# wreuven/h264-scroll-encoder

Hardware: AMD Instinct MI355X
Metric: composed frames/sec (1280x720, 360x360 dyn) at 1/2/4/8 GPU; bit-exact vs CPU (higher is better)
Workload: dtype u8; 1 GPU; BASELINE config 3: 256 concurrent 1280x720 streams + 360x360 synthetic dynamic rect (4x4 int transform + quant + CAVLC), composer_write_scroll_frame semantics; resolution=1280x720, streams_per_gpu=256, parallelism=static stream shard x1, no RCCL

## Files before the change

### h264-scroll-encoder_amd/csrc/dyn_kernels.hip

```cpp
#include <hip/hip_runtime.h>

#include <stdint.h>
#include <mutex>

#include "dyn_device.h"
#include "dyn_engine.h"
#include "nal_ctx.h"
#include "stage_util.h"

using namespace scroll;
using namespace scroll::dyn;
using namespace scroll::stage;

namespace {

__constant__ Tabs g_tabs = SCROLL_DYN_TABS;
constexpr Tabs k_tabs = SCROLL_DYN_TABS;
__constant__ PTabs g_ptabs = make_ptabs(k_tabs);
__device__ uint32_t g_tzrb[TZRB_N];
struct QpPair {
    QParams l, c;
};
struct QpTab {
    QpPair q[QP_MAX + 1];
};
constexpr QpTab make_qptab()
{
    QpTab T{};
    for (int i = 0; i <= QP_MAX; ++i) T.q[i] = QpPair{qparams(i), qparams(qp_chroma(i))};
// ... 4 lines not shown
__global__ __launch_bounds__(256) void k_tzrb_init()
{
    const int i = blockIdx.x * 256 + threadIdx.x;
    if (i < TZRB_N) g_tzrb[i] = i < 65536 ? tzrb_entry(g_tabs, (uint32_t)i, 16) : tzrb_entry(g_tabs, (uint32_t)(i - 65536), 15);
}

__device__ inline void load_ptabs(PTabs &dst, int t, int nthr)
{
    constexpr int N = (int)(sizeof(PTabs) / 16);
    static_assert(sizeof(PTabs) % 16 == 0, "PTabs copies as uint4");
    for (int i = t; i < N; i += nthr) reinterpret_cast<uint4 *>(&dst)[i] = reinterpret_cast<const uint4 *>(&g_ptabs)[i];
}

constexpr int HEAD_MAX = 160;
constexpr int HDR_MAX = 1024;
constexpr int OBUF = 6400;

constexpr uint32_t DF_OVER = 1u, DF_GENERAL = 2u, DF_HANDOFF = 4u;
constexpr uint64_t HANDOFF_TICKS = 5000000ull;
constexpr uint64_t HANDOFF_GAP = 100000ull;
constexpr uint32_t DF_EPSLOW = 0x100u;
constexpr uint32_t DF_FIXED = 0x200u;

constexpr int EPC_ROW = 256, EPC_STATIC = 4096;

__device__ inline uint32_t ep_data(uint32_t w, uint32_t gi, uint32_t bits)
{
    const uint32_t b0 = 32u * gi;
    if (__builtin_expect(b0 + 32u <= bits, 1)) return w;
    return w | (bits > b0 ? 0xffffffffu >> (bits - b0) : 0xffffffffu);
}

__device__ inline uint32_t ep_run_starts(uint32_t pw, uint32_t w, uint32_t nx, uint32_t gi, uint32_t bits)
{
    uint64_t X = (uint64_t)ep_data(w, gi, bits) << 32 | ep_data(nx, gi + 1u, bits);
    X |= X << 1;
    X |= X << 2;
    X |= X << 4;
    X |= X << 8;
    X |= X << 6;
    const uint32_t z22 = ~(uint32_t)(X >> 32);
    return z22 & ((ep_data(w, gi, bits) >> 1) | (pw << 31));
}

__device__ inline bool ep_quick(uint32_t w, uint32_t nx)
{
    uint32_t y = w | w << 1;
    y |= y << 2;
    y |= y << 4;
    y |= y << 8;
    y |= y << 6;
    const uint32_t tz = w ? (uint32_t)__builtin_ctz(w) : 32u, lz = nx ? (uint32_t)__builtin_clz(nx) : 32u;
    return (~y & 0xffe00000u) != 0u || tz + lz >= 22u;
}

__device__ inline void flush_window(const uint32_t *buf, uint32_t n, uint32_t p0, bool last, uint32_t *out,
                                    uint32_t *ncand, uint32_t *cg, uint32_t cmax, int t, int nthr)
{
    const int lane = t & 63;
    for (uint32_t i0 = 0; i0 < n; i0 += (uint32_t)nthr) {
        const uint32_t i = i0 + (uint32_t)t;
        bool q = false;
        if (i < n) {
            const uint32_t w = buf[i];
            out[p0 + i] = w;
            q = ep_quick(w, i + 1 < n ? buf[i + 1] : (last ? 0xffffffffu : 0u));
        }
        const uint64_t m = __builtin_amdgcn_ballot_w64(q);
        if (m) {
            uint32_t base = 0;
            if (lane == (int)__builtin_ctzll(m)) base = atomicAdd(ncand, (uint32_t)__builtin_popcountll(m));
            base = (uint32_t)__shfl((int)base, (int)__builtin_ctzll(m), 64);
            const uint32_t k = base + (uint32_t)__builtin_popcountll(m & ((1ull << lane) - 1ull));
            if (q && k < cmax) cg[1 + k] = p0 + i;
        }
    }
}

__device__ inline uint32_t ld32(const uint8_t *p) { return *reinterpret_cast<const uint32_t *>(p); }

constexpr int NPC = DYN_PIECES;

__device__ inline void put_body(uint2 *BL, uint2 *BH, size_t i, uint4 v, bool hi)
{
    BL[i] = make_uint2(v.x, v.y);
    if (hi) BH[i] = make_uint2(v.z, v.w);
}

__device__ inline uint4 get_body(const uint2 *BL, const uint2 *BH, size_t i, bool hi)
{
    const uint2 a = BL[i], b = hi ? BH[i] : make_uint2(0u, 0u);
    return make_uint4(a.x, a.y, b.x, b.y);
}

__device__ inline int rec_of(int q, int pc, int ndt)
{
    return pc < 16 ? 16 * q + pc : (pc < 18 ? 24 * ndt + 2 * q + (pc - 16) : 16 * ndt + 8 * q + (pc - 18));
// ... 562 lines not shown
        uint32_t e = 0u;
        if (gen) {
            const uint32_t k = atomicAdd(&ctr[1], 1u);
            if (k < g.gen_cap) {
                DF->rbsp_bytes = k;
                ctr[DYN_CTR_LIST + k] = (uint32_t)((size_t)s * ld_fr + f);
                e = DF_GENERAL;
            } else {
                e = DF_OVER;
            }
        }
        DF->err = e;
        DF->ep = (uint32_t)qpy;
    }
}

constexpr int GW = 64;
#ifndef SCROLL_GBUF_WORDS
#define SCROLL_GBUF_WORDS 256
#endif
constexpr int GBUF_WORDS = SCROLL_GBUF_WORDS;

struct StaticFixed {
    uint32_t ncand;
    uint32_t buf[GBUF_WORDS];
    uint64_t hhi[12], hlo[12];
    uint4 pat[12];
    uint32_t hlen[12];
    int32_t head_over;
    int32_t wo[8], wl[8], wv[8];
    uint32_t moff[DYN_STATIC_ROWS + 1];
};

__global__ __launch_bounds__(GW) void k_dyn_static(const DevStream *__restrict__ st,
                                                   const NalDesc *__restrict__ nal, int ld_nal,
                                                   const PlanPending *__restrict__ pend,
                                                   const DynFrame *__restrict__ dfr, int ld_fr, DynGeom g,
                                                   uint32_t *__restrict__ rowstage, uint32_t *__restrict__ gbits)
{
    __shared__ StaticFixed L;
    constexpr int SR = DYN_STATIC_ROWS;
    const Rect R{g.x0, g.y0, g.w, g.h};
    const int nA = max(1, (R.y0 + SR - 1) / SR);
    const int gi = (int)blockIdx.x >= nA ? (int)blockIdx.x + R.h : (int)blockIdx.x;
    const int ng = g.ngroups, f = blockIdx.y, s = blockIdx.z, t = threadIdx.x;
    const size_t nb = (size_t)s * ld_fr + f;
    const DynFrame df = dfr[nb];
    const int j = df.nal;
    if (j < 0) return;
    const bool first = gi == 0, last = gi == ng - 1;
    if (t < 8) {
        L.wo[t] = pend[s].wo[t];
        L.wl[t] = pend[s].wl[t];
        L.wv[t] = pend[s].wv[t];
    }
    if (t == 0) {
        L.head_over = 0;
        L.ncand = 0;
    }
    const DevStream *S = st + s;
    const NalDesc d = nal[(size_t)s * ld_nal + j];
    wave_sync();
    NalCtx c = nal_ctx(S, d, L.wo, L.wl, L.wv);
    c.qpd = (int)df.ep - QP_DEFAULT;
    const HeadCtx H = head_ctx(c);
    const int mbw = H.mbw, mbh = c.h / 16;
    int ra, rb;
    if (gi < nA) {
        ra = gi * SR;
        rb = min(ra + SR, R.y0);
    } else {
        ra = R.y0 + R.h + (gi - nA - R.h) * SR;
        rb = min(ra + SR, mbh);
    }
    uint32_t F = 0;
    if (first) {
        CountSink hc{0};
        emit_slice_header(hc, c);
        F = hc.n;
    }
    if (t < 12) {
// ... 97 lines not shown
                    const uint32_t w0 = wi == 0 ? P.x : (wi == 1 ? P.y : (wi == 2 ? P.z : P.w));
                    const uint32_t w1 = wi == 0 ? P.y : (wi == 1 ? P.z : (wi == 2 ? P.w : 0u));
                    uint32_t v = sh ? __builtin_amdgcn_alignbit(w0, w1, 32u - sh) : w0;
                    v &= k >= 32u ? 0xffffffffu : ~(0xffffffffu >> k);
                    acc |= v >> (b - W0);
                    b += k;
                }
                L.buf[i] = acc;
            }
            wave_sync();
            if (first && t == 0 && p0 * 32u < F) {
                WSink hs{win, 0, 0, 0};
                hs.start(0);
                emit_slice_header(hs, c);
                hs.finish();
            }
            if (last && t == 0) {
                WSink sk{win, 0, 0, 0};
                sk.start(bits - 1u);
                sk.put(1, 1);
                sk.finish();
            }
            wave_sync();
            flush_window(L.buf, n, p0, p0 + n >= nw, out, &L.ncand,
                         rowstage + nb * g.rs_frame_words + rs_runs_words(g, nA, gi), EPC_STATIC - 1, t, GW);
            wave_sync();
            continue;
        }
        const int ea = max(cnt_le(32u * p0) - 1, 0), eb = min(cnt_le(32u * (p0 + n) - 1u), ne);
        const int nm = eb * mbw;
        for (int m = ea * mbw + t; m < nm; m += GW) {
            const int rr = (int)div_m((uint32_t)m, m_mbw), col = m - rr * mbw, rw = ra + rr;
            uint32_t off = L.moff[rr];
            WSink sk{win, 0, 0, 0};
            if (!head_over) {
                const int b3 = H.sel(rw, 0);
                off += col == 0 ? 0u : L.hlen[b3] + 1u + (uint32_t)(col - 1) * (L.hlen[b3 + 1] + 1u);
                if (off >= 32u * (p0 + n)) continue;
                const int cls = b3 + (col == 0 ? 0 : (col == mbw - 1 ? 2 : 1));
                if (off + L.hlen[cls] + 1u <= 32u * p0) continue;
                sk.start(off);
                sk.put_cap(CapSink{L.hhi[cls], L.hlo[cls], L.hlen[cls]});
            } else {
                for (int c2 = 0; c2 < col; ++c2) off += head_bits(rw, c2) + 1u;
                sk.start(off);
                H.put_slow(sk, rw, col);
            }
            sk.put(1, 1);
            sk.finish();
        }
        if (last && t == 0) {
            WSink sk{win, 0, 0, 0};
            sk.start(bits - 1u);
            sk.put(1, 1);
            sk.finish();
        }
        wave_sync();
        flush_window(L.buf, n, p0, p0 + n >= nw, out, &L.ncand,
                     rowstage + nb * g.rs_frame_words + rs_runs_words(g, nA, gi), EPC_STATIC - 1, t, GW);
        wave_sync();
    }
    if (t == 0) rowstage[nb * g.rs_frame_words + rs_runs_words(g, nA, gi)] = L.ncand;
}


__device__ inline CapSink cap_of_msb(uint64_t a, uint64_t b, uint32_t n)
{
    if (n == 0u) return CapSink{0, 0, 0};
    const uint32_t sh = 128u - n;
    if (sh >= 64u) return CapSink{0, a >> (sh - 64u), n};
    if (sh == 0u) return CapSink{a, b, n};
    return CapSink{a >> sh, (b >> sh) | (a << (64u - sh)), n};
}

__device__ inline void put_piece(uint32_t *buf, uint32_t p0, uint32_t n, uint32_t pos, uint32_t tv, uint32_t tl,
                                 uint4 b, uint32_t bl)
{
    const uint32_t tw = tv & low_mask((int)tl);
    const uint32_t c0 = __builtin_amdgcn_alignbit(tw, b.x, tl), c1 = __builtin_amdgcn_alignbit(b.x, b.y, tl);
    const uint32_t c2 = __builtin_amdgcn_alignbit(b.y, b.z, tl), c3 = __builtin_amdgcn_alignbit(b.z, b.w, tl);
    const uint32_t c4 = __builtin_amdgcn_alignbit(b.w, 0u, tl);
    const uint32_t sh = pos & 31u;
    const uint32_t o[6] = {c0 >> sh, __builtin_amdgcn_alignbit(c0, c1, sh), __builtin_amdgcn_alignbit(c1, c2, sh),
                           __builtin_amdgcn_alignbit(c2, c3, sh), __builtin_amdgcn_alignbit(c3, c4, sh),
                           __builtin_amdgcn_alignbit(c4, 0u, sh)};
// ... 43 lines not shown
#define SCROLL_ROW_GB 896
#endif
constexpr int ROW_GB = SCROLL_ROW_GB;

constexpr int ROW_PCD_N = (NPC + 3) & ~3;

struct RowFixed {
    RowTabs ptabs;
    uint32_t pcd[ROW_PCD_N];
    union {
        uint32_t buf[ROW_GB + 4];
        struct {
            uint32_t kc[2][SORT_KEYS];
            uint32_t ovf;
            uint32_t kc_pad[31 - 2 * SORT_KEYS];
            uint32_t lvt[LVT_N];
        };
    };
    uint64_t hhi[12], hlo[12];
    uint32_t hlen[12];
    int32_t wo[8], wl[8], wv[8];
    int32_t head_over;
    uint32_t rt[32];
    uint32_t ncand;
    uint32_t spill;
};

static_assert(2 * SORT_KEYS < 31 && 32 + LVT_N <= ROW_GB, "the sort counts, ovf and the level table share the bit window");
static_assert(ROW_PAD == 4, "RowFixed::buf holds ROW_PAD spare words");
static_assert(sizeof(RowFixed) <= 4992, "eight config-3 row workgroups per CU");

__host__ __device__ inline size_t row_lds_base(int w)
{
    return (size_t)16 * NPC * w + (size_t)4 * (w + 1) + (size_t)2 * (3 * NPC * w) + (size_t)10 * w + 16;
}
#ifndef SCROLL_ROW_GB_WIDE
#define SCROLL_ROW_GB_WIDE 1248
#endif
constexpr int ROW_GB_WIDE = SCROLL_ROW_GB_WIDE;
__host__ __device__ inline size_t row_wide_off(int w) { return (row_lds_base(w) + 15) & ~(size_t)15; }
__host__ __device__ inline bool row_wide_win(int w)
{
    return w > SCROLL_ROW_WIDE && row_wide_off(w) + 4 * (size_t)(ROW_GB_WIDE + ROW_PAD) + sizeof(RowFixed) <= 163840;
}
__host__ __device__ inline size_t row_lds_bytes(int w)
{
    return row_wide_win(w) ? row_wide_off(w) + 4 * (size_t)(ROW_GB_WIDE + ROW_PAD) : row_lds_base(w);
// ... 33 lines not shown
    RowConst C{};
    const PTabs P = make_ptabs(T);
    for (int i = 0; i < 4 * 68; ++i) C.ptabs.ct[i / 68][i % 68] = P.ct[i / 68][i % 68];
    for (int i = 0; i < 12; ++i) C.ptabs.tzdc[i / 4][i % 4] = P.tzdc[i / 4][i % 4];
    for (int i = 0; i < 7 * 16; ++i) C.ptabs.rb[i / 16][i % 16] = P.rb[i / 16][i % 16];
    for (int i = 0; i < NPC; ++i) C.pcd[i] = pc_desc(i);
    const LvTab V = make_lvt();
    for (int i = 0; i < LVT_N; ++i) C.lvt[i] = V.e[i];
    return C;
}
__constant__ RowConst g_rowconst = make_rowconst(k_tabs);
constexpr int ROWC_NV = (int)(sizeof(RowConst) / 16), ROWC_HEAD = (int)(offsetof(RowConst, lvt) / 16);
constexpr int ROWC_GAP = (int)((offsetof(RowFixed, lvt) - offsetof(RowConst, lvt)) / 16);
static_assert(offsetof(RowFixed, ptabs) == 0 && offsetof(RowFixed, pcd) == offsetof(RowConst, pcd) &&
                  offsetof(RowFixed, kc) == offsetof(RowConst, lvt) && offsetof(RowFixed, lvt) % 16 == 0 &&
                  sizeof(RowConst) % 16 == 0 && sizeof(RowConst) == 16 * ROWC_HEAD + 4 * LVT_N,
              "RowConst is RowFixed's head without the sort's words");
static_assert(offsetof(RowFixed, wl) == offsetof(RowFixed, wo) + 32 && offsetof(RowFixed, wv) == offsetof(RowFixed, wo) + 64 &&
                  offsetof(PlanPending, wl) == offsetof(PlanPending, wo) + 32 &&
                  offsetof(PlanPending, wv) == offsetof(PlanPending, wo) + 64,
              "the waypoint table copies as 24 words");

struct EpfLds {
    uint32_t *goff, *gb, *gw, *cw, *cbase, *lst, *cnt;
    uint32_t *ws;
};
__host__ __device__ inline int row_chroma0(int w) { return (16 * w + 63) & ~63; }
__host__ __device__ inline int row_vtasks(int w) { return row_chroma0(w) + 8 * w; }

__host__ __device__ inline int row_threads(int w)
{
    const int nt = row_vtasks(w), np = w > SCROLL_ROW_WIDE ? SCROLL_ROW_NP_WIDE : SCROLL_ROW_NP;
    const int a = (((nt + np - 1) / np) + 63) & ~63;
    const int b = (((nt + ROW_NPMAX - 1) / ROW_NPMAX) + 63) & ~63;
    const int t = a > b ? a : b;
    return t < ROW_MAXT ? t : ROW_MAXT;
}

struct BlkPix {
    uint32_t a[4], b[4], c;
};

__device__ inline __amdgpu_buffer_rsrc_t buf_rsrc(const void *p, uint32_t n)
{
    return __builtin_amdgcn_make_buffer_rsrc(const_cast<void *>(p), (short)0, (int)n, 0x00020000);
}

// ... 171 lines not shown
        const uint32_t rtv = rtg[e < 16 ? 16 * r + e : 16 * g.h + (e < 24 ? 8 * r + e - 16 : 8 * g.h + 8 * r + e - 24)];
        if (k0 == 0) {
            fetch_luma(fo, t, r, g, rtg + 16 * r);
            fo.pb = 0;
            fetch_pass9(fo, 0u, (uint32_t)(16 * w), fs, rb, nx);
            nx.c = 0u;
            L.rt[e] = rtv;
        } else if (k0 == 1) {
            fetch_chroma(fo, t - L0, r, g, csz, rtg + 16 * g.h + 8 * r, rtg + 24 * g.h + 8 * r);
            fo.pb = 0;
            fo_chroma = true;
            fetch_pass9(fo, 0u, (uint32_t)(8 * w), fs, rb, nx);
        }
    }
    if (df.nal < 0 || ((df.err & DF_GENERAL) != 0) != GEN) return;

    uint4 *lv = rdyn;
    uint32_t *moff = reinterpret_cast<uint32_t *>(lv + npc);
    uint16_t *mt = reinterpret_cast<uint16_t *>(moff + w + 1), *lo = mt + npc, *off16 = lo + npc;
    uint16_t *order = off16;
    uint8_t *ta = reinterpret_cast<uint8_t *>(off16 + npc), *cbpa = ta + 8 * w, *codea = cbpa + w;
    uint32_t *mbits = reinterpret_cast<uint32_t *>(ta);

    if (t == 0) L.ncand = 0;
    if (t == 0) L.ovf = 0u;
    if (t < SORT_KEYS) L.kc[0][t] = 0u;
    if (general && wv0 == T - 64) row_copy_tabs(L, s, nb, lane);
    const int qpy = __builtin_amdgcn_readfirstlane((int)df.ep);
    const QParams ql = g_qptab.q[qpy].l, qc = g_qptab.q[qpy].c;
    const HeadSel HS = head_sel(S, a.nal[(size_t)s * a.ld_nal + df.nal]);
    if (!general)
        asm volatile(""
                     :
                     : "s"(HS.a_end), "s"(HS.mbw), "s"(ql.mf0), "s"(ql.mf1), "s"(ql.mf2), "s"(ql.qbits), "s"(ql.qf),
                       "s"(qc.mf0), "s"(qc.mf1), "s"(qc.mf2), "s"(qc.qbits), "s"(qc.qf));

    __syncthreads();
    if (!general) {
        static_assert(ROW_MAXT % 64 == 0, "row_threads gives whole waves: the per-pass step T is a multiple of 64");
        const uint32_t frc = __builtin_amdgcn_readfirstlane((L.rt[16] >> 28) & 7u);
        const int qL = nl > wv0 ? (nl - wv0 + T - 1) / T : 0;
        const int qC = ntv > wv0 ? (ntv - wv0 + T - 1) / T : 0;
        auto issue_l = [&](int q, BlkPix &px) {
            fetch_pass9(fo, (uint32_t)((q - fo.pb) * T), (uint32_t)(16 * w), fs, rb, px);
        };
        auto issue_c = [&](int q, BlkPix &px) {
            if (!fo_chroma) {
// ... 472 lines not shown
            const uint32_t o = off16[i];
            if (o == 0xffffu) continue;
            const int k = div_npc(i), pc = i - k * NPC;
            const uint32_t e = lo[i], mv = mt[i];
            const uint32_t pos = moff[k] + o;
            if (!one && (pos >= 32u * (p0 + n) || pos + (e & LO_LEN) <= 32u * p0)) continue;
            const int nC = (int)(e >> 11) - 1;
            const uint4 bd = lv[i];
            if (!(mv & M_OVF)) {
                if (nC == -1) {
                    if (one) put_piece1(wb, pos, 0u, 0u, bd, e & LO_LEN);
                    else put_piece(wb, p0, n, pos, 0u, 0u, bd, e & LO_LEN);
                } else {
                    uint32_t tv = 0, tl = 0;
                    piece_token(ctab, mv, nC, tv, tl);
                    if (one) put_piece1(wb, pos, tv, tl, bd, mv & 255u);
                    else put_piece(wb, p0, n, pos, tv, tl, bd, mv & 255u);
                }
            } else {
                ovf_put((LdsWords)wb, p0, n, pos, PT, TB, bd, ovf_wide(k, pc), pc, nC);
            }
        }
        __syncthreads();
        flush_window(wb, n, p0, p0 + n >= nw, out, &L.ncand, out + epc, EPC_ROW - 1, t, T);
        __syncthreads();
    }
    if (t == 0 && !lost) out[epc] = L.ncand;
    if (stp && t == 0) {
        stp[5] = __builtin_amdgcn_s_memrealtime();
        stp[6] = bits;
        stp[7] = (uint64_t)(uint32_t)__builtin_amdgcn_s_getreg((31 << 11) | 4);
    }
}

#ifndef SCROLL_EPS_KW
#define SCROLL_EPS_KW 4
#endif
constexpr int EPS_KW = SCROLL_EPS_KW;
static_assert(EPS_KW % 4 == 0, "the EP scan reads 16-byte LDS vectors");
__host__ __device__ inline size_t gtab_bytes(int ng, bool epfix)
{
    return (size_t)4 * (epfix ? 5 * (size_t)ng + 2 : 3 * (size_t)ng + 1);
}
struct GTab {
    uint32_t *goff, *gb, *gw, *cw, *cbase;
};
__device__ inline GTab gtab_of(uint32_t *p, int ng)
{
    GTab T;
    T.goff = p;
    T.gb = p + ng + 1;
    T.gw = T.gb + ng;
    T.cw = T.gw + ng;
    T.cbase = T.cw + ng;
    return T;
}

__device__ inline uint32_t rs_word_span(uint32_t P, int &gg, int ng, uint32_t T, const uint32_t *goff,
                                       const uint32_t *gb, const uint32_t *gw, const uint32_t *fr)
{
    uint32_t acc = 0, filled = 0;
    while (filled < 32u && gg < ng && P + filled < T) {
        const uint32_t lp = P + filled - goff[gg];
        if (lp >= gb[gg]) {
            ++gg;
            continue;
        }
        const uint32_t take = min(32u - filled, gb[gg] - lp);
        const uint32_t *src = fr + gw[gg];
        const uint32_t i = lp >> 5, sh = lp & 31u;
        uint32_t x = src[i];
        if (sh) {
            x <<= sh;
            if (32u - sh < take) x |= src[i + 1] >> (32u - sh);
        }
        x &= take >= 32u ? 0xffffffffu : ~(0xffffffffu >> take);
        acc |= x >> filled;
// ... 22 lines not shown
__device__ inline void scan_load(ScanLoads &L, uint32_t c0, int t, int ng, uint32_t T, const uint32_t *goff,
                                   const uint32_t *gb, const uint32_t *gw, const uint32_t *fr, int &gcarry)
{
    const uint32_t P0 = c0 * 8u + 32u * (uint32_t)t;
    int gg = gcarry;
    while (gg + 1 < ng && goff[gg + 1] <= P0) ++gg;
#pragma unroll
    for (int k = 0; k < EPS_KW; ++k) {
        const uint32_t P = P0 + 32u * NT * (uint32_t)k;
        while (gg + 1 < ng && goff[gg + 1] <= P) ++gg;
        L.g[k] = gg;
        const uint32_t lp = P - goff[gg], i = lp >> 5;
        const uint32_t *src = fr + gw[gg];
        L.x0[k] = P < T && lp < gb[gg] ? src[i] : 0u;
        L.x1[k] = P < T && (lp & 31u) && 32u * (i + 1) < gb[gg] ? src[i + 1] : 0u;
        const bool seam = P < T && gb[gg] - lp < 32u && gg + 1 < ng;
        L.y[k] = seam ? fr[gw[gg + 1]] : 0u;
    }
    gcarry = gg;
}

__device__ inline void rs_table(const uint32_t *gbits, size_t nb, const DynGeom &g, const uint32_t *fr,
                                uint32_t *goff, uint32_t *gb, uint32_t *gw, uint32_t *cw, int t,
                                uint32_t *bad = nullptr, uint32_t *cnt = nullptr)
{
    const int ng = g.ngroups;
    constexpr int SR = DYN_STATIC_ROWS;
    const int nA = max(1, (g.y0 + SR - 1) / SR);
    if (t >= 64) return;
    uint32_t carry = 0;
    for (int g0 = 0; g0 < ng; g0 += 64) {
        const int gi = g0 + t;
        const bool in = gi < ng;
        const bool row = gi >= nA && gi < nA + g.h;
        uint32_t w = (uint32_t)rs_group_words(g, nA, gi), c = (uint32_t)rs_runs_words(g, nA, gi);
        const uint32_t b = in ? gbits[nb * (size_t)ng + gi] : 0u;
        uint32_t m = in && (row || cnt) ? fr[c] : 0u;
        const uint32_t incl = wave_incl_sum(b, t);
        if (in) {
            gb[gi] = b;
            goff[gi] = carry + incl - b;
            if (row && (m & 0x80000000u)) {
                const uint64_t base = ((uint64_t)g.rs_frames - nb) * g.rs_frame_words;
                const uint64_t rel = (uint64_t)(m & 0x7fffffffu) - base;
                if ((m & 0x7fffffffu) >= base && rel % g.rs_spill_words == 0 &&
                    rel / g.rs_spill_words < g.rs_spill_cap) {
                    w = m & 0x7fffffffu;
                    c = w + g.rs_spill_words - EPC_ROW;
                    if (cnt) m = fr[c];
                } else {
                    if (bad) *bad = 1u;
                    m = 0u;
                }
            }
            gw[gi] = w;
            if (cw) cw[gi] = c;
            if (cnt) cnt[gi] = m;
        }
        carry += __shfl(incl, 63, 64);
    }
    if (t == 0) goff[ng] = carry;
}

__device__ inline uint32_t rs_word(uint32_t P, int ng, uint32_t T, const uint32_t *goff, const uint32_t *gb,
                                   const uint32_t *gw, const uint32_t *fr)
{
    if (P >= T) return 0u;
    int gg = rs_group_at(P, ng, goff);
    return rs_word_span(P, gg, ng, T, goff, gb, gw, fr);
}

__device__ inline uint32_t pick9(const uint32_t w[9], uint32_t i)
{
    const uint32_t a = (i & 1u) ? w[1] : w[0], b = (i & 1u) ? w[3] : w[2];
    const uint32_t c = (i & 1u) ? w[5] : w[4], e = (i & 1u) ? w[7] : w[6];
    const uint32_t ab = (i & 2u) ? b : a, ce = (i & 2u) ? e : c;
    const uint32_t r = (i & 4u) ? ce : ab;
    return (i & 8u) ? w[8] : r;
}

// ... 147 lines not shown
    }
    __syncthreads();
    return ep_n;
}

#ifndef SCROLL_EPF_T
#define SCROLL_EPF_T 128
#endif
#ifndef SCROLL_EPF_LIST
#define SCROLL_EPF_LIST 2048
#endif
constexpr int EPF_T = SCROLL_EPF_T;

__device__ inline void ep_put(uint32_t j, bool bm, uint32_t *lst, uint32_t *nlst, uint32_t lcap)
{
    if (bm) {
        atomicOr(&lst[j >> 5], 1u << (j & 31u));
    } else {
        const uint32_t q = atomicAdd(nlst, 1u);
        if (q < lcap) lst[q] = j;
    }
}

__device__ inline void ep_eval_bytes(uint32_t B, uint32_t Bend, uint32_t nin, int ng, uint32_t T,
                                     const uint32_t *goff, const uint32_t *gb, const uint32_t *gw,
                                     const uint32_t *fr, bool bm, uint32_t *lst, uint32_t *nlst, uint32_t lcap)
{
    uint32_t cw = 0, ci = 0xffffffffu;
    auto byte_at = [&](uint32_t i) -> uint32_t {
        if ((i >> 2) != ci) {
            ci = i >> 2;
            cw = rs_word(32u * ci, ng, T, goff, gb, gw, fr);
        }
        return (cw >> (8u * (3u - (i & 3u)))) & 255u;
    };
    int k = 0;
    for (int64_t i = (int64_t)B - 1; i >= 0; --i) {
        if (byte_at((uint32_t)i)) break;
        ++k;
    }
    for (uint32_t i = B; i < nin; ++i) {
        const uint32_t b = byte_at(i);
        if (ep_insert(b, k)) ep_put(i, bm, lst, nlst, lcap);
        if (b == 0) {
            ++k;
        } else {
            if (i >= Bend) break;
            k = 0;
        }
    }
}

__device__ inline int cand_group(uint32_t i, int ng, const uint32_t *cbase)
{
    int lo = 0, hi = ng;
    while (hi - lo > 1) {
        const int mid = (lo + hi) >> 1;
        if (cbase[mid] <= i) lo = mid;
        else hi = mid;
    }
    return lo;
}

template <int NT, int LCAP>
__device__ __attribute__((always_inline)) inline uint32_t ep_list_windows(uint32_t *lst, uint32_t n, uint32_t nin,
                                                                          uint32_t *eplist, uint32_t *ws, int t,
                                                                          int lane, int wave, uint32_t ecap)
{
    const uint32_t ws0 = (n + 4u * NT - 1u) / (4u * NT) * (4u * NT);
    const uint32_t HW = (uint32_t)LCAP - ws0, CH = HW / (uint32_t)NT;
    uint32_t *win = lst + ws0;
    const uint4 *wv = reinterpret_cast<const uint4 *>(win) + (uint32_t)t * (CH / 4u);
    uint32_t base = 0;
    for (uint32_t w0 = 0; w0 < nin; w0 += 32u * HW) {
        for (uint32_t i = (uint32_t)t; i < HW / 4u; i += (uint32_t)NT)
            reinterpret_cast<uint4 *>(win)[i] = make_uint4(0u, 0u, 0u, 0u);
// ... 20 lines not shown
        ex += incl - mine;
        for (uint32_t k = 0; mine && k < CH / 4u; ++k) {
            const uint4 q = wv[k];
            const uint32_t wv4[4] = {q.x, q.y, q.z, q.w};
#pragma unroll
            for (int e = 0; e < 4; ++e)
                for (uint32_t m = wv4[e]; m; m &= m - 1u) {
                    if (ex < ecap)
                        eplist[ex] = w0 + 32u * ((uint32_t)t * CH + 4u * k + (uint32_t)e) + (uint32_t)__builtin_ctz(m);
                    ++ex;
                }
        }
        base += tot;
        __syncthreads();
    }
    return base;
}

template <int NT, int LCAP>
__device__ inline void ep_fix(DevStream *st, DynFrame *DF, size_t nb, int s, const DynGeom &g,
                              const uint32_t *rowstage, const uint32_t *gbits, uint8_t *eps, const EpfLds &E,
                              int t, uint64_t *stp)
{
    static_assert(NT >= 128 && NT % 64 == 0, "ep_fix: one seam wave and at least one candidate wave");
    static_assert(LCAP % (4 * NT) == 0 && LCAP >= 8 * NT, "ep_fix: the bitmap in whole 16-byte chunks per thread");
    auto stamp = [&](int k) {
        if (stp && t == 0) stp[k] = __builtin_amdgcn_s_memrealtime();
    };
    stamp(0);
    uint32_t *goff = E.goff, *gb = E.gb, *gw = E.gw, *cw = E.cw, *cbase = E.cbase, *lst = E.lst;
    uint32_t &nlst = E.cnt[0], &nu = E.cnt[1], &slow = E.cnt[2], &bad = E.cnt[3];
    const uint32_t lcap = LCAP;
    const uint32_t err0 = DF->err;
    if (err0 & (DF_OVER | DF_HANDOFF)) {
        if (t == 0) {
            DF->rbsp_bytes = 0;
            DF->ep = 0;
            DF->err = err0 | DF_FIXED;
            atomicOr((unsigned int *)&st[s].err,
                     (err0 & DF_HANDOFF) ? SCROLL_DEVERR_HANDOFF : SCROLL_DEVERR_DYN);
        }
        return;
    }
    const int ng = g.ngroups;
    constexpr int SR = DYN_STATIC_ROWS;
    const int nA = max(1, (g.y0 + SR - 1) / SR);
    const uint32_t *fr = rowstage + nb * g.rs_frame_words;
    for (uint32_t i = (uint32_t)t; i < lcap / 4u; i += (uint32_t)NT)
        reinterpret_cast<uint4 *>(lst)[i] = make_uint4(0u, 0u, 0u, 0u);
    if (t < 64) {
        if (t == 0) bad = 0u;
        wave_sync();
        rs_table(gbits, nb, g, fr, goff, gb, gw, cw, t, &bad, cbase);
        wave_sync();
        uint32_t carry = 0;
        bool ov = false;
        for (int g0 = 0; g0 < ng; g0 += 64) {
            const int gi = g0 + t;
            const uint32_t c = gi < ng ? cbase[gi] : 0u;
            const uint32_t cmax = (gi >= nA && gi < nA + g.h) ? EPC_ROW - 1u : EPC_STATIC - 1u;
            const uint32_t cc = min(c, cmax);
            const uint32_t incl = wave_incl_sum(cc, t);
            if (gi < ng) cbase[gi] = carry + incl - cc;
            ov |= __builtin_amdgcn_ballot_w64(c > cmax) != 0;
            carry += __shfl(incl, 63, 64);
        }
        if (t == 0) {
            cbase[ng] = carry;
            slow = ov ? 1u : 0u;
            nlst = 0;
        }
    }
    __syncthreads();
    stamp(1);
    if (bad) {
        if (t == 0) {
            DF->err = DF_OVER | DF_FIXED;
            DF->rbsp_bytes = 0;
            DF->ep = 0;
            atomicOr((unsigned int *)&st[s].err, SCROLL_DEVERR_DYN);
        }
        return;
    }
    const uint32_t T = goff[ng];
    const uint32_t nin = (T + 7) >> 3;
    if (((nin + 31u) & ~31u) > g.slot_bytes - DYN_OVF_BYTES) {
        if (t == 0) {
            DF->err = DF_OVER | DF_FIXED;
            DF->rbsp_bytes = 0;
            DF->ep = 0;
            atomicOr((unsigned int *)&st[s].err, SCROLL_DEVERR_DYN);
        }
        return;
    }
    const uint32_t nbw = (nin + 31u) >> 5;
    const bool bm = nbw <= lcap;
    const int wave = t >> 6, lane = t & 63;
    constexpr int NC = NT;
    const uint32_t nc = cbase[ng];
    if (!slow) {
        if (wave == NT / 64 - 1) {
            for (int k = lane; k < ng; k += 64) {
                const uint32_t S = goff[k];
                if (S < T) ep_eval_bytes(S >> 3, (S + 7) >> 3, nin, ng, T, goff, gb, gw, fr, bm, lst, &nlst, lcap);
            }
            if (stp && lane == 0) stp[7] = __builtin_amdgcn_s_memrealtime();
        }
        constexpr int CB = NC >= 192 ? 2 : 4;
        for (uint32_t i0 = 0; i0 < nc; i0 += (uint32_t)(CB * NC)) {
            uint32_t wi[CB], gg[CB];
#pragma unroll
            for (int q = 0; q < CB; ++q) {
                const uint32_t ci = i0 + (uint32_t)(q * NC + t);
                gg[q] = ci < nc ? (uint32_t)cand_group(ci, ng, cbase) : 0u;
                wi[q] = ci < nc ? fr[cw[gg[q]] + 1u + (ci - cbase[gg[q]])] : 0xffffffffu;
            }
            uint32_t pw[CB], w[CB], nx[CB], nwd[CB];
#pragma unroll
            for (int q = 0; q < CB; ++q) {
                const uint32_t *src = fr + gw[gg[q]];
                nwd[q] = (gb[gg[q]] + 31u) >> 5;
                const bool ok = wi[q] < nwd[q];
                pw[q] = ok && wi[q] ? src[wi[q] - 1u] : 0u;
                w[q] = ok ? src[wi[q]] : 0u;
                nx[q] = ok && wi[q] + 1u < nwd[q] ? src[wi[q] + 1u] : 0u;
            }
#pragma unroll
            for (int q = 0; q < CB; ++q) {
                if (wi[q] >= nwd[q]) continue;
                const uint32_t bits = gb[gg[q]], O = goff[gg[q]], x = wi[q];
                const uint32_t *src = fr + gw[gg[q]];
                const uint32_t wd = ep_data(w[q], x, bits);
                const uint32_t nd = x + 1u < nwd[q] ? ep_data(nx[q], x + 1u, bits) : 0xffffffffu;
                uint32_t m = ep_run_starts(pw[q], wd, nd, x, bits);
                while (m) {
                    const uint32_t a = (uint32_t)__builtin_clz(m);
                    m &= ~(0x80000000u >> a);
                    const uint64_t Y = ((uint64_t)wd << 32 | nd) << a;
                    uint32_t e = bits;
                    if (Y) {
                        e = 32u * x + a + (uint32_t)__builtin_clzll(Y);
                    } else {
                        for (uint32_t r = x + 2u; r < nwd[q]; ++r) {
                            const uint32_t v = ep_data(src[r], r, bits);
                            if (v) {
                                e = 32u * r + (uint32_t)__builtin_clz(v);
                                break;
                            }
                        }
                    }
                    const uint32_t A = (O + 32u * x + a + 7u) & ~7u, E2 = O + e;
                    for (uint32_t j = A + 16u; j + 6u <= E2; j += 16u) ep_put(j >> 3, bm, lst, &nlst, lcap);
                }
            }
        }
        stamp(4);
    }
    __syncthreads();
    stamp(2);
    const uint32_t n = nlst;
    uint32_t *eplist = reinterpret_cast<uint32_t *>(eps + nb * eps_stride(g));
    if (slow || (!bm && n > lcap)) {
        static_assert(NT * EPS_KW <= LCAP, "ep_scan's chunk buffer is the position set's LDS");
        __syncthreads();
        const uint32_t ne = ep_scan<NT>(fr, ng, T, goff, gb, gw, lst, reinterpret_cast<int *>(E.ws), nlst, eplist, t, g.ep_cap);
        if (t == 0) {
            DF->err = DF_EPSLOW | DF_FIXED;
            DF->rbsp_bytes = nin;
            DF->ep = ne;
        }
        return;
    }
    constexpr int CW = LCAP / NT;
    if (!bm && n <= lcap - 4u * NT) {
        const uint32_t base = ep_list_windows<NT, LCAP>(lst, n, nin, eplist, E.ws, t, lane, wave, g.ep_cap);
        stamp(3);
// ... 81 lines not shown
#endif
#if SCROLL_EPF_WAVES
#define EPF_ATTR __attribute__((amdgpu_waves_per_eu(SCROLL_EPF_WAVES)))
#else
#define EPF_ATTR
#endif
template <int NT, int LCAP>
__global__ __launch_bounds__(NT) EPF_ATTR void k_dyn_epfix(DevStream *__restrict__ st, DynFrame *__restrict__ dfr,
                                                     int ld_fr, int nframes, DynGeom g,
                                                     const uint32_t *__restrict__ rowstage,
                                                     const uint32_t *__restrict__ gbits, uint8_t *__restrict__ eps,
                                                     uint64_t *__restrict__ stamps)
{
    __shared__ __attribute__((aligned(16))) uint32_t lst[LCAP];
    extern __shared__ uint32_t gdyn[];
    const GTab GT = gtab_of(gdyn, g.ngroups);
    uint32_t *goff = GT.goff, *gb = GT.gb, *gw = GT.gw, *cw = GT.cw, *cbase = GT.cbase;
    __shared__ uint32_t cnt[4], ws[NT / 64];
    const int f = blockIdx.x, s = blockIdx.y, t = threadIdx.x;
    if (f >= nframes) return;
    const size_t nb = (size_t)s * ld_fr + f;
    DynFrame *DF = dfr + nb;
    if (DF->nal < 0) return;
    const EpfLds E{goff, gb, gw, cw, cbase, lst, cnt, ws};
    ep_fix<NT, LCAP>(st, DF, nb, s, g, rowstage, gbits, eps, E, t, stamps ? stamps + ((size_t)s * nframes + f) * 8 : nullptr);
}
constexpr int EPF_BIG_LIST = 8192;
constexpr int EPF_BIG_MBS = 1024;
inline bool epf_big_rect(int64_t mbs)
{
    static const int env = [] {
        const char *e = getenv("SCROLL_EPF_BIG");
        return e ? atoi(e) : -1;
    }();
    return env >= 0 ? env != 0 : mbs > EPF_BIG_MBS;
}

__device__ inline void store16(uint8_t *A, uint64_t p, const uint8_t *src, uint64_t lo, uint64_t hi)
{
    if (p >= lo && p + 16 <= hi) {
        *reinterpret_cast<uint4 *>(A + p) = *reinterpret_cast<const uint4 *>(src);
        return;
    }
    for (int i = 0; i < 16; ++i)
        if (p + i >= lo && p + i < hi) A[p + i] = src[i];
}

// ... 796 lines not shown
```

Before: 3.253 million frames/s.

## Record run edges and candidate words in emulation-prevention records to skip byte-scan seams

Emulation-prevention candidate records now store each candidate's word and next word, plus per-group leading and trailing zero-run lengths, written where the rows and static groups are encoded. The fix kernel then handles group seams as precomputed zero runs spread across all threads, instead of one wave walking bytes serially through rs_word. Most candidates also no longer re-read their neighbouring bitstream words. In exchange, candidate records are three times larger, the LDS table grows, and the seam logic is more intricate and must stay bit-exact.

```diff
diff --git a/h264-scroll-encoder_amd/csrc/dyn_kernels.hip b/h264-scroll-encoder_amd/csrc/dyn_kernels.hip
--- a/h264-scroll-encoder_amd/csrc/dyn_kernels.hip
+++ b/h264-scroll-encoder_amd/csrc/dyn_kernels.hip
@@ -5,6 +5,7 @@
 
 #include "dyn_device.h"
 #include "dyn_engine.h"
+#include "ep_runs.h"
 #include "nal_ctx.h"
 #include "stage_util.h"
 
@@ -55,57 +56,39 @@
 constexpr uint32_t DF_EPSLOW = 0x100u;
 constexpr uint32_t DF_FIXED = 0x200u;
 
-constexpr int EPC_ROW = 256, EPC_STATIC = 4096;
-
-__device__ inline uint32_t ep_data(uint32_t w, uint32_t gi, uint32_t bits)
-{
-    const uint32_t b0 = 32u * gi;
-    if (__builtin_expect(b0 + 32u <= bits, 1)) return w;
-    return w | (bits > b0 ? 0xffffffffu >> (bits - b0) : 0xffffffffu);
-}
-
-__device__ inline uint32_t ep_run_starts(uint32_t pw, uint32_t w, uint32_t nx, uint32_t gi, uint32_t bits)
-{
-    uint64_t X = (uint64_t)ep_data(w, gi, bits) << 32 | ep_data(nx, gi + 1u, bits);
-    X |= X << 1;
-    X |= X << 2;
-    X |= X << 4;
-    X |= X << 8;
-    X |= X << 6;
-    const uint32_t z22 = ~(uint32_t)(X >> 32);
-    return z22 & ((ep_data(w, gi, bits) >> 1) | (pw << 31));
-}
-
-__device__ inline bool ep_quick(uint32_t w, uint32_t nx)
-{
-    uint32_t y = w | w << 1;
-    y |= y << 2;
-    y |= y << 4;
-    y |= y << 8;
-    y |= y << 6;
-    const uint32_t tz = w ? (uint32_t)__builtin_ctz(w) : 32u, lz = nx ? (uint32_t)__builtin_clz(nx) : 32u;
-    return (~y & 0xffe00000u) != 0u || tz + lz >= 22u;
-}
+constexpr int EPC_ROW_N = 255, EPC_STATIC_N = 4095;
+constexpr int EPC_ROW = (int)(EPR_HDR + EPR_ENTRY * EPC_ROW_N), EPC_STATIC = (int)(EPR_HDR + EPR_ENTRY * EPC_STATIC_N);
+
+struct EpRec {
+    uint32_t n, open;
+};
 
 __device__ inline void flush_window(const uint32_t *buf, uint32_t n, uint32_t p0, bool last, uint32_t *out,
-                                    uint32_t *ncand, uint32_t *cg, uint32_t cmax, int t, int nthr)
+                                    EpRec *rec, uint32_t *cg, uint32_t cmax, int t, int nthr)
 {
     const int lane = t & 63;
+    if (t == 0) ep_window_edges(buf, n, p0, &rec->open, &cg[1]);
     for (uint32_t i0 = 0; i0 < n; i0 += (uint32_t)nthr) {
         const uint32_t i = i0 + (uint32_t)t;
         bool q = false;
         if (i < n) {
-            const uint32_t w = buf[i];
-            out[p0 + i] = w;
-            q = ep_quick(w, i + 1 < n ? buf[i + 1] : (last ? 0xffffffffu : 0u));
+            out[p0 + i] = buf[i];
+            q = ep_window_quick(buf, n, last, i);
         }
         const uint64_t m = __builtin_amdgcn_ballot_w64(q);
         if (m) {
             uint32_t base = 0;
-            if (lane == (int)__builtin_ctzll(m)) base = atomicAdd(ncand, (uint32_t)__builtin_popcountll(m));
+            if (lane == (int)__builtin_ctzll(m)) base = atomicAdd(&rec->n, (uint32_t)__builtin_popcountll(m));
             base = (uint32_t)__shfl((int)base, (int)__builtin_ctzll(m), 64);
             const uint32_t k = base + (uint32_t)__builtin_popcountll(m & ((1ull << lane) - 1ull));
-            if (q && k < cmax) cg[1 + k] = p0 + i;
+            if (q && k < cmax) {
+                uint32_t e[EPR_ENTRY];
+                ep_cand_entry(buf, n, p0, last, i, e);
+                uint32_t *dst = cg + EPR_HDR + EPR_ENTRY * k;
+                dst[0] = e[0];
+                dst[1] = e[1];
+                dst[2] = e[2];
+            }
         }
     }
 }
@@ -714,7 +697,7 @@
 constexpr int GBUF_WORDS = SCROLL_GBUF_WORDS;
 
 struct StaticFixed {
-    uint32_t ncand;
+    EpRec epr;
     uint32_t buf[GBUF_WORDS];
     uint64_t hhi[12], hlo[12];
     uint4 pat[12];
@@ -748,7 +731,7 @@
     }
     if (t == 0) {
         L.head_over = 0;
-        L.ncand = 0;
+        L.epr = EpRec{0u, 0u};
     }
     const DevStream *S = st + s;
     const NalDesc d = nal[(size_t)s * ld_nal + j];
@@ -892,8 +875,8 @@
                 sk.finish();
             }
             wave_sync();
-            flush_window(L.buf, n, p0, p0 + n >= nw, out, &L.ncand,
-                         rowstage + nb * g.rs_frame_words + rs_runs_words(g, nA, gi), EPC_STATIC - 1, t, GW);
+            flush_window(L.buf, n, p0, p0 + n >= nw, out, &L.epr,
+                         rowstage + nb * g.rs_frame_words + rs_runs_words(g, nA, gi), EPC_STATIC_N, t, GW);
             wave_sync();
             continue;
         }
@@ -926,11 +909,11 @@
             sk.finish();
         }
         wave_sync();
-        flush_window(L.buf, n, p0, p0 + n >= nw, out, &L.ncand,
-                     rowstage + nb * g.rs_frame_words + rs_runs_words(g, nA, gi), EPC_STATIC - 1, t, GW);
+        flush_window(L.buf, n, p0, p0 + n >= nw, out, &L.epr,
+                     rowstage + nb * g.rs_frame_words + rs_runs_words(g, nA, gi), EPC_STATIC_N, t, GW);
         wave_sync();
     }
-    if (t == 0) rowstage[nb * g.rs_frame_words + rs_runs_words(g, nA, gi)] = L.ncand;
+    if (t == 0) ep_record_close(rowstage + nb * g.rs_frame_words + rs_runs_words(g, nA, gi), L.epr.n, L.epr.open, bits);
 }
 
 
@@ -1020,7 +1003,7 @@
     int32_t wo[8], wl[8], wv[8];
     int32_t head_over;
     uint32_t rt[32];
-    uint32_t ncand;
+    EpRec epr;
     uint32_t spill;
 };
 
@@ -1100,7 +1083,7 @@
               "the waypoint table copies as 24 words");
 
 struct EpfLds {
-    uint32_t *goff, *gb, *gw, *cw, *cbase, *lst, *cnt;
+    uint32_t *goff, *gb, *gw, *cw, *cbase, *lead, *trail, *lst, *cnt;
     uint32_t *ws;
 };
 __host__ __device__ inline int row_chroma0(int w) { return (16 * w + 63) & ~63; }
@@ -1318,7 +1301,7 @@
     uint8_t *ta = reinterpret_cast<uint8_t *>(off16 + npc), *cbpa = ta + 8 * w, *codea = cbpa + w;
     uint32_t *mbits = reinterpret_cast<uint32_t *>(ta);
 
-    if (t == 0) L.ncand = 0;
+    if (t == 0) L.epr = EpRec{0u, 0u};
     if (t == 0) L.ovf = 0u;
     if (t < SORT_KEYS) L.kc[0][t] = 0u;
     if (general && wv0 == T - 64) row_copy_tabs(L, s, nb, lane);
@@ -1837,10 +1820,10 @@
             }
         }
         __syncthreads();
-        flush_window(wb, n, p0, p0 + n >= nw, out, &L.ncand, out + epc, EPC_ROW - 1, t, T);
+        flush_window(wb, n, p0, p0 + n >= nw, out, &L.epr, out + epc, EPC_ROW_N, t, T);
         __syncthreads();
     }
-    if (t == 0 && !lost) out[epc] = L.ncand;
+    if (t == 0 && !lost) ep_record_close(out + epc, L.epr.n, L.epr.open, bits);
     if (stp && t == 0) {
         stp[5] = __builtin_amdgcn_s_memrealtime();
         stp[6] = bits;
@@ -1855,10 +1838,10 @@
 static_assert(EPS_KW % 4 == 0, "the EP scan reads 16-byte LDS vectors");
 __host__ __device__ inline size_t gtab_bytes(int ng, bool epfix)
 {
-    return (size_t)4 * (epfix ? 5 * (size_t)ng + 2 : 3 * (size_t)ng + 1);
+    return (size_t)4 * (epfix ? 7 * (size_t)ng + 2 : 3 * (size_t)ng + 1);
 }
 struct GTab {
-    uint32_t *goff, *gb, *gw, *cw, *cbase;
+    uint32_t *goff, *gb, *gw, *cw, *cbase, *lead, *trail;
 };
 __device__ inline GTab gtab_of(uint32_t *p, int ng)
 {
@@ -1868,6 +1851,8 @@
     T.gw = T.gb + ng;
     T.cw = T.gw + ng;
     T.cbase = T.cw + ng;
+    T.lead = T.cbase + ng + 1;
+    T.trail = T.lead + ng;
     return T;
 }
 
@@ -1936,7 +1921,8 @@
 
 __device__ inline void rs_table(const uint32_t *gbits, size_t nb, const DynGeom &g, const uint32_t *fr,
                                 uint32_t *goff, uint32_t *gb, uint32_t *gw, uint32_t *cw, int t,
-                                uint32_t *bad = nullptr, uint32_t *cnt = nullptr)
+                                uint32_t *bad = nullptr, uint32_t *cnt = nullptr, uint32_t *lead = nullptr,
+                                uint32_t *trail = nullptr)
 {
     const int ng = g.ngroups;
     constexpr int SR = DYN_STATIC_ROWS;
@@ -1950,6 +1936,7 @@
         uint32_t w = (uint32_t)rs_group_words(g, nA, gi), c = (uint32_t)rs_runs_words(g, nA, gi);
         const uint32_t b = in ? gbits[nb * (size_t)ng + gi] : 0u;
         uint32_t m = in && (row || cnt) ? fr[c] : 0u;
+        uint32_t lz = in && cnt ? fr[c + 1u] : 0u, tz = in && cnt ? fr[c + 2u] : 0u;
         const uint32_t incl = wave_incl_sum(b, t);
         if (in) {
             gb[gi] = b;
@@ -1961,7 +1948,11 @@
                     rel / g.rs_spill_words < g.rs_spill_cap) {
                     w = m & 0x7fffffffu;
                     c = w + g.rs_spill_words - EPC_ROW;
-                    if (cnt) m = fr[c];
+                    if (cnt) {
+                        m = fr[c];
+                        lz = fr[c + 1u];
+                        tz = fr[c + 2u];
+                    }
                 } else {
                     if (bad) *bad = 1u;
                     m = 0u;
@@ -1969,7 +1960,11 @@
             }
             gw[gi] = w;
             if (cw) cw[gi] = c;
-            if (cnt) cnt[gi] = m;
+            if (cnt) {
+                cnt[gi] = m;
+                lead[gi] = min(lz, b);
+                trail[gi] = min(tz, b);
+            }
         }
         carry += __shfl(incl, 63, 64);
     }
@@ -2163,36 +2158,7 @@
     }
 }
 
-__device__ inline void ep_eval_bytes(uint32_t B, uint32_t Bend, uint32_t nin, int ng, uint32_t T,
-                                     const uint32_t *goff, const uint32_t *gb, const uint32_t *gw,
-                                     const uint32_t *fr, bool bm, uint32_t *lst, uint32_t *nlst, uint32_t lcap)
-{
-    uint32_t cw = 0, ci = 0xffffffffu;
-    auto byte_at = [&](uint32_t i) -> uint32_t {
-        if ((i >> 2) != ci) {
-            ci = i >> 2;
-            cw = rs_word(32u * ci, ng, T, goff, gb, gw, fr);
-        }
-        return (cw >> (8u * (3u - (i & 3u)))) & 255u;
-    };
-    int k = 0;
-    for (int64_t i = (int64_t)B - 1; i >= 0; --i) {
-        if (byte_at((uint32_t)i)) break;
-        ++k;
-    }
-    for (uint32_t i = B; i < nin; ++i) {
-        const uint32_t b = byte_at(i);
-        if (ep_insert(b, k)) ep_put(i, bm, lst, nlst, lcap);
-        if (b == 0) {
-            ++k;
-        } else {
-            if (i >= Bend) break;
-            k = 0;
-        }
-    }
-}
-
-__device__ inline int cand_group(uint32_t i, int ng, const uint32_t *cbase)
+__device__ inline int entry_group(uint32_t i, int ng, const uint32_t *cbase)
 {
     int lo = 0, hi = ng;
     while (hi - lo > 1) {
@@ -2259,7 +2225,7 @@
                               const uint32_t *rowstage, const uint32_t *gbits, uint8_t *eps, const EpfLds &E,
                               int t, uint64_t *stp)
 {
-    static_assert(NT >= 128 && NT % 64 == 0, "ep_fix: one seam wave and at least one candidate wave");
+    static_assert(NT >= 128 && NT % 64 == 0, "ep_fix: whole waves, two at least");
     static_assert(LCAP % (4 * NT) == 0 && LCAP >= 8 * NT, "ep_fix: the bitmap in whole 16-byte chunks per thread");
     auto stamp = [&](int k) {
         if (stp && t == 0) stp[k] = __builtin_amdgcn_s_memrealtime();
@@ -2288,14 +2254,16 @@
     if (t < 64) {
         if (t == 0) bad = 0u;
         wave_sync();
-        rs_table(gbits, nb, g, fr, goff, gb, gw, cw, t, &bad, cbase);
+        rs_table(gbits, nb, g, fr, goff, gb, gw, cw, t, &bad, cbase, E.lead, E.trail);
         wave_sync();
         uint32_t carry = 0;
         bool ov = false;
         for (int g0 = 0; g0 < ng; g0 += 64) {
             const int gi = g0 + t;
             const uint32_t c = gi < ng ? cbase[gi] : 0u;
-            const uint32_t cmax = (gi >= nA && gi < nA + g.h) ? EPC_ROW - 1u : EPC_STATIC - 1u;
+            const uint32_t cmax = (g.debug & SCROLL_DEBUG_DYN_EPCAP4)
+                                      ? 0u
+                                      : (uint32_t)((gi >= nA && gi < nA + g.h) ? EPC_ROW_N : EPC_STATIC_N);
             const uint32_t cc = min(c, cmax);
             const uint32_t incl = wave_incl_sum(cc, t);
             if (gi < ng) cbase[gi] = carry + incl - cc;
@@ -2333,62 +2301,52 @@
     const uint32_t nbw = (nin + 31u) >> 5;
     const bool bm = nbw <= lcap;
     const int wave = t >> 6, lane = t & 63;
-    constexpr int NC = NT;
     const uint32_t nc = cbase[ng];
     if (!slow) {
-        if (wave == NT / 64 - 1) {
-            for (int k = lane; k < ng; k += 64) {
-                const uint32_t S = goff[k];
-                if (S < T) ep_eval_bytes(S >> 3, (S + 7) >> 3, nin, ng, T, goff, gb, gw, fr, bm, lst, &nlst, lcap);
-            }
-            if (stp && lane == 0) stp[7] = __builtin_amdgcn_s_memrealtime();
-        }
-        constexpr int CB = NC >= 192 ? 2 : 4;
-        for (uint32_t i0 = 0; i0 < nc; i0 += (uint32_t)(CB * NC)) {
-            uint32_t wi[CB], gg[CB];
+        constexpr int CB = 2;
+        const uint32_t nseam = (uint32_t)ng + 1u, nitem = nseam + nc;
+        auto put = [&](uint32_t j) { ep_put(j, bm, lst, &nlst, lcap); };
+        for (uint32_t i0 = 0; i0 < nitem; i0 += (uint32_t)(CB * NT)) {
+            uint32_t ex[CB], ew[CB], en[CB];
+            int gq[CB];
 #pragma unroll
             for (int q = 0; q < CB; ++q) {
-                const uint32_t ci = i0 + (uint32_t)(q * NC + t);
-                gg[q] = ci < nc ? (uint32_t)cand_group(ci, ng, cbase) : 0u;
-                wi[q] = ci < nc ? fr[cw[gg[q]] + 1u + (ci - cbase[gg[q]])] : 0xffffffffu;
-            }
-            uint32_t pw[CB], w[CB], nx[CB], nwd[CB];
+                const uint32_t i = i0 + (uint32_t)(q * NT + t);
+                gq[q] = -1;
+                ex[q] = ew[q] = en[q] = 0u;
+                if (i >= nseam && i < nitem) {
+                    const uint32_t ci = i - nseam;
+                    gq[q] = entry_group(ci, ng, cbase);
+                    const uint32_t *r = fr + cw[gq[q]] + EPR_HDR + EPR_ENTRY * (ci - cbase[gq[q]]);
+                    ex[q] = r[0];
+                    ew[q] = r[1];
+                    en[q] = r[2];
+                }
+            }
+            if (stp && t == 0 && i0 == 0) {
+                __builtin_amdgcn_s_waitcnt(0);
+                stp[7] = __builtin_amdgcn_s_memrealtime();
+            }
 #pragma unroll
             for (int q = 0; q < CB; ++q) {
-                const uint32_t *src = fr + gw[gg[q]];
-                nwd[q] = (gb[gg[q]] + 31u) >> 5;
-                const bool ok = wi[q] < nwd[q];
-                pw[q] = ok && wi[q] ? src[wi[q] - 1u] : 0u;
-                w[q] = ok ? src[wi[q]] : 0u;
-                nx[q] = ok && wi[q] + 1u < nwd[q] ? src[wi[q] + 1u] : 0u;
-            }
-#pragma unroll
-            for (int q = 0; q < CB; ++q) {
-                if (wi[q] >= nwd[q]) continue;
-                const uint32_t bits = gb[gg[q]], O = goff[gg[q]], x = wi[q];
-                const uint32_t *src = fr + gw[gg[q]];
-                const uint32_t wd = ep_data(w[q], x, bits);
-                const uint32_t nd = x + 1u < nwd[q] ? ep_data(nx[q], x + 1u, bits) : 0xffffffffu;
-                uint32_t m = ep_run_starts(pw[q], wd, nd, x, bits);
-                while (m) {
-                    const uint32_t a = (uint32_t)__builtin_clz(m);
-                    m &= ~(0x80000000u >> a);
-                    const uint64_t Y = ((uint64_t)wd << 32 | nd) << a;
-                    uint32_t e = bits;
-                    if (Y) {
-                        e = 32u * x + a + (uint32_t)__builtin_clzll(Y);
-                    } else {
-                        for (uint32_t r = x + 2u; r < nwd[q]; ++r) {
-                            const uint32_t v = ep_data(src[r], r, bits);
-                            if (v) {
-                                e = 32u * r + (uint32_t)__builtin_clz(v);
-                                break;
-                            }
-                        }
-                    }
-                    const uint32_t A = (O + 32u * x + a + 7u) & ~7u, E2 = O + e;
-                    for (uint32_t j = A + 16u; j + 6u <= E2; j += 16u) ep_put(j >> 3, bm, lst, &nlst, lcap);
+                const uint32_t i = i0 + (uint32_t)(q * NT + t);
+                if (i < nseam) {
+                    uint32_t rs = 0, re = 0;
+                    if (ep_seam_run((int)i, ng, goff, gb, E.lead, E.trail, rs, re)) ep_run_positions(rs, re, put);
+                    continue;
                 }
+                if (gq[q] < 0) continue;
+                const uint32_t bits = gb[gq[q]], O = goff[gq[q]], x = ex[q] & EPR_IDX;
+                const uint32_t *src = fr + gw[gq[q]];
+                const uint32_t nwd = (bits + 31u) >> 5;
+                bool pw = (ex[q] & EPR_PW) != 0u;
+                if ((ex[q] & EPR_DATA) && x < nwd) {
+                    pw = x && (src[x - 1u] & 1u);
+                    ew[q] = src[x];
+                    en[q] = x + 1u < nwd ? src[x + 1u] : 0u;
+                }
+                ep_cand_runs(x, pw, ew[q], en[q], bits, [&](uint32_t r) { return src[r]; },
+                             [&](uint32_t a, uint32_t e) { ep_run_positions(O + a, O + e, put); });
             }
         }
         stamp(4);
@@ -2516,7 +2474,7 @@
     const size_t nb = (size_t)s * ld_fr + f;
     DynFrame *DF = dfr + nb;
     if (DF->nal < 0) return;
-    const EpfLds E{goff, gb, gw, cw, cbase, lst, cnt, ws};
+    const EpfLds E{goff, gb, gw, cw, cbase, GT.lead, GT.trail, lst, cnt, ws};
     ep_fix<NT, LCAP>(st, DF, nb, s, g, rowstage, gbits, eps, E, t, stamps ? stamps + ((size_t)s * nframes + f) * 8 : nullptr);
 }
 constexpr int EPF_BIG_LIST = 8192;
diff --git a/h264-scroll-encoder_amd/csrc/ep_runs.h b/h264-scroll-encoder_amd/csrc/ep_runs.h
--- /dev/null
+++ b/h264-scroll-encoder_amd/csrc/ep_runs.h
@@ -0,0 +1,132 @@
+#pragma once
+#include <cstdint>
+
+#if !defined(__HIPCC__) && !defined(__device__)
+#define __device__
+#define __host__
+#endif
+
+namespace scroll {
+namespace dyn {
+
+constexpr uint32_t EPR_MIN = 22u;
+
+constexpr uint32_t EPR_HDR = 3u, EPR_ENTRY = 3u;
+constexpr uint32_t EPR_PW = 0x80000000u, EPR_DATA = 0x40000000u, EPR_IDX = 0x00ffffffu;
+
+__host__ __device__ inline uint32_t ep_data(uint32_t w, uint32_t gi, uint32_t bits)
+{
+    const uint32_t b0 = 32u * gi;
+    if (__builtin_expect(b0 + 32u <= bits, 1)) return w;
+    return w | (bits > b0 ? 0xffffffffu >> (bits - b0) : 0xffffffffu);
+}
+
+__host__ __device__ inline uint32_t ep_run_starts(uint32_t pw, uint32_t w, uint32_t nx)
+{
+    uint64_t X = (uint64_t)w << 32 | nx;
+    X |= X << 1;
+    X |= X << 2;
+    X |= X << 4;
+    X |= X << 8;
+    X |= X << 6;
+    const uint32_t z22 = ~(uint32_t)(X >> 32);
+    return z22 & ((w >> 1) | (pw << 31));
+}
+
+__host__ __device__ inline bool ep_quick(uint32_t w, uint32_t nx)
+{
+    uint32_t y = w | w << 1;
+    y |= y << 2;
+    y |= y << 4;
+    y |= y << 8;
+    y |= y << 6;
+    const uint32_t tz = w ? (uint32_t)__builtin_ctz(w) : 32u, lz = nx ? (uint32_t)__builtin_clz(nx) : 32u;
+    return (~y & 0xffe00000u) != 0u || tz + lz >= EPR_MIN;
+}
+
+template <class Put>
+__host__ __device__ inline void ep_run_positions(uint32_t S, uint32_t E, Put &&put)
+{
+    const uint32_t A = (S + 7u) & ~7u;
+    for (uint32_t j = A + 16u; j + 6u <= E; j += 16u) put(j >> 3);
+}
+
+__host__ __device__ inline bool ep_window_quick(const uint32_t *buf, uint32_t n, bool last, uint32_t i)
+{
+    return ep_quick(buf[i], i + 1u < n ? buf[i + 1u] : (last ? 0xffffffffu : 0u));
+}
+
+__host__ __device__ inline void ep_cand_entry(const uint32_t *buf, uint32_t n, uint32_t p0, bool last, uint32_t i,
+                                              uint32_t e[EPR_ENTRY])
+{
+    const bool edge = (i == 0u && p0 > 0u) || (i + 1u == n && !last);
+    e[0] = (p0 + i) | (i && (buf[i - 1u] & 1u) ? EPR_PW : 0u) | (edge ? EPR_DATA : 0u);
+    e[1] = buf[i];
+    e[2] = i + 1u < n ? buf[i + 1u] : 0u;
+}
+
+__host__ __device__ inline void ep_window_edges(const uint32_t *buf, uint32_t n, uint32_t p0, uint32_t *open,
+                                                uint32_t *lead)
+{
+    uint32_t wf = buf[0], wl = buf[n - 1u];
+    const uint32_t o = *open;
+    uint32_t i = 0, k = n - 1u;
+    while (!wf && ++i < n) wf = buf[i];
+    if (!wf) return;
+    if (o == 0u) *lead = 32u * (p0 + i) + (uint32_t)__builtin_clz(wf);
+    while (!wl) wl = buf[--k];
+    *open = 32u * (p0 + k) + 32u - (uint32_t)__builtin_ctz(wl);
+}
+
+__host__ __device__ inline void ep_record_close(uint32_t *rec, uint32_t cnt, uint32_t open, uint32_t bits)
+{
+    rec[0] = cnt;
+    if (open == 0u) rec[1] = bits;
+    rec[2] = bits - open;
+}
+
+template <class Word, class Emit>
+__host__ __device__ inline void ep_cand_runs(uint32_t x, bool pw, uint32_t w, uint32_t nx, uint32_t bits,
+                                             Word &&word, Emit &&emit)
+{
+    const uint32_t nw = (bits + 31u) >> 5;
+    if (x >= nw) return;
+    const uint32_t wd = ep_data(w, x, bits), nd = x + 1u < nw ? ep_data(nx, x + 1u, bits) : 0xffffffffu;
+    uint32_t m = ep_run_starts(x && pw ? 1u : 0u, wd, nd);
+    while (m) {
+        const uint32_t a = (uint32_t)__builtin_clz(m);
+        m &= ~(0x80000000u >> a);
+        const uint64_t Y = ((uint64_t)wd << 32 | nd) << a;
+        uint32_t e = bits;
+        if (Y) {
+            e = 32u * x + a + (uint32_t)__builtin_clzll(Y);
+        } else {
+            for (uint32_t r = x + 2u; r < nw; ++r) {
+                const uint32_t v = ep_data(word(r), r, bits);
+                if (v) {
+                    e = 32u * r + (uint32_t)__builtin_clz(v);
+                    break;
+                }
+            }
+        }
+        if (e < bits) emit(32u * x + a, e);
+    }
+}
+
+__host__ __device__ inline bool ep_seam_run(int k, int ng, const uint32_t *goff, const uint32_t *gb,
+                                            const uint32_t *lead, const uint32_t *trail, uint32_t &S, uint32_t &E)
+{
+    if (k == 0) {
+        S = 0u;
+    } else {
+        if (lead[k - 1] >= gb[k - 1]) return false;
+        S = goff[k] - trail[k - 1];
+    }
+    int j = k;
+    while (j < ng && lead[j] >= gb[j]) ++j;
+    E = j < ng ? goff[j] + lead[j] : (goff[ng] + 7u) & ~7u;
+    return true;
+}
+
+}
+}
```

After: 3.258 million frames/s, median of 6. No clear change (+0.2%).
